# liangxuy/ReGenNet

Measured on AMD Instinct MI355X. Metric: sampled motions/sec, higher is better.
Workload: dtype bf16 MFMA operands, fp32 accumulate/LayerNorm/softmax, for 990 of 1000 steps; fp16 MFMA operands for the next 8; split-bf16 (x3) for the last 2; 1 GPU; ntu: [B=256/GPU,56,6,60] online/concat/no_cond L8 d512, 1000-step DDPM, Philox noise, hipGraph=on; batch_per_gpu=256, global_batch=256, denoiser_evals_per_motion=1000, parallelism=batch-shard x1

## Files before the change

regennet_amd/csrc/rgn_layers.hip:

```cpp
#include "rgn_internal.h"
#include "rgn_device.h"
#include "rgn_tail.h"
#include "rgn_sampler.h"

#include <hip/hip_runtime.h>

#include <cmath>
#include <type_traits>
#include <utility>

namespace rgn {

#ifndef RGN_LY_ST_AUX
#define RGN_LY_ST_AUX 16
#endif

constexpr int LY_NTH = 512, LY_KB = 4096;
constexpr int LY_X = 0, LY_Y = 64 * 1024, LY_EXCH = LY_Y, LY_RED = 128 * 1024, LY_REDF = 2 * 8 * 64, LY_VEC = LY_RED + 2 * LY_REDF * 4, LY_VECW = 640,
              LY_LDS = 160 * 1024;
constexpr int LY_PF = LY_VEC + 8 * LY_VECW * 4;
static_assert(LY_PF + 8 * 256 <= LY_LDS, "LDS map");
enum { V_BO = 0, V_G1 = 64, V_G2 = 128, V_B2 = 192, V_SPV = 256, V_BF1 = 320 , V_BF2 = 448, V_G3 = 512, V_B3 = 576 };
constexpr int LY_RDA = 6;
constexpr int LY_RDM = 8;
struct LYT {
    static constexpr int MT = 2, NT = 2, NW = 8, R = 64, RD = LY_RDM, KB = LY_KB, RED = LY_RED, REDF = LY_REDF;
};

#ifdef RGN_LY_STAMPS
__device__ long long g_ly_st[1024][16];
#define RGN_LYT(i)                                                                                   \
    {                                                                                                \
        __builtin_amdgcn_sched_barrier(0);                                                           \
        if (threadIdx.x == 0 && blockIdx.x < 1024 && l == RGN_LY_STAMPS) g_ly_st[blockIdx.x][i] = __builtin_readcyclecounter(); \
        __builtin_amdgcn_sched_barrier(0);                                                           \
    }
#define RGN_LYS(i)                                                                                   \
    {                                                                                                \
        __builtin_amdgcn_sched_barrier(0);                                                           \
        if (threadIdx.x == 0 && blockIdx.x < 1024 && it == 1) g_ly_st[blockIdx.x][i] = __builtin_readcyclecounter(); \
        __builtin_amdgcn_sched_barrier(0);                                                           \
    }
#else
#define RGN_LYT(i)
#define RGN_LYS(i)
#endif

constexpr int LY_XLD = 356, LY_TILE = 0, LY_XIMG = 92160, LY_NKX = 11;
static_assert(64 * LY_XLD * 4 <= LY_XIMG && LY_XIMG + LY_NKX * 4096 <= LY_LDS, "step boundary LDS map");

template <bool STEPS, bool GUIDED = false, bool F16 = false, bool INPAINT = false>
__global__ __launch_bounds__(LY_NTH, 2) void k_layers(LayersArgs g) {
    static_assert(STEPS || !GUIDED, "guidance inside the launch needs the step boundary");
    static_assert(STEPS || !INPAINT, "in-painting (rgn_set_inpainting) belongs to the step boundary");
    using OP = OpFmt<F16>;
    using op_t = typename OP::t;
    using op8 = typename OP::v8;
    using op4 = typename OP::v4;
    extern __shared__ __attribute__((aligned(16))) char smem[];
    const int tid = threadIdx.x, lane = tid & 63;
    const int wave = __builtin_amdgcn_readfirstlane(tid >> 6);
    const int wn = wave & 3, hg = wave >> 2;
    const int l31 = lane & 31, kh = lane >> 5;
    const int b = xcd_affine(blockIdx.x, gridDim.x), Tq = g.Tq;
    const size_t row0 = (size_t)b * Tq;
#ifdef RGN_LY_PRIO
    if (wave >= 4) __builtin_amdgcn_s_setprio(RGN_LY_PRIO);
#endif
    float* vec = reinterpret_cast<float*>(smem + LY_VEC) + wave * LY_VECW;
    const int lane16 = lane * 16;
    tile_dma_in(smem + LY_X, g.h, g.rows, row0, Tq, lane, wave);
    const int first_step = (g.stepvec || STEPS) ? *g.d_step : 0;
    const TailLane tl = tail_lane<LYT>(smem, lane, wave);
    static_assert(LY_X == 0, "a_off addresses the image at byte 0");
    int a_off[2], a_offy[2];
    tail_a_off(a_off, lane);
    tail_a_off(a_offy, a_off, LY_Y);
    using Pass = TailPass;
    op8 wf[LY_RDM][2];
    const float qs2 = g.qscale * 1.44269504088896340736f;

    f32x4 qb[4];
    float vb1;
    auto load_qbias = [&](const float* bqkv, int r) {
        const float* bq = bqkv + (2 * r + hg) * 128 + wn * 32;
#pragma unroll
        for (int i4 = 0; i4 < 4; ++i4) qb[i4] = *reinterpret_cast<const f32x4*>(bq + 8 * i4 + 4 * kh);
        vb1 = bq[1024 + l31];
    };

    wait_vmcnt<0>();
    __builtin_amdgcn_s_barrier();
    load_qbias(g.lw[0].bqkv, 0);

    const int nit = STEPS ? g.steps : 1;
    auto out_proj = [&](f32x16 (&acc)[2][2], int wv) {
#pragma unroll
        for (int a2 = 0; a2 < 2; ++a2)
#pragma unroll
            for (int b2 = 0; b2 < 2; ++b2)
#pragma unroll
                for (int i = 0; i < 16; ++i) acc[a2][b2][i] = 0.f;
        if (wv < 6) {
            const int cb0 = 2 * wv;
            const Pass p_out{__builtin_amdgcn_make_buffer_rsrc(const_cast<__bf16*>(g.Wout) + (size_t)cb0 * 1024, 0, (16 * g.nb_out - cb0) * 2048, 0x00020000), LY_NKX * 2048, 0};
#pragma unroll
            for (int s2 = 0; s2 < LY_RDM - 1; ++s2) tail_load_g<OP, LYT>(wf, tl, p_out, s2, s2);
            tail_gemm<OP, LYT, 32, false, 0>(acc, wf, tl, a_off, p_out, p_out);
        }
    };
    for (int it = 0; it < nit; ++it) {
    const int step = first_step - it;
    for (int pass = 0; pass < (GUIDED ? 2 : 1); ++pass) {
    if (GUIDED && pass == 1) {
        f32x16 accp[2][2];
        int wave_p = wave, lane_p = lane, b_p = b;
        asm volatile("" : "+s"(wave_p), "+s"(b_p));
        asm volatile("" : "+v"(lane_p));
        out_proj(accp, wave_p);
        if (wave_p < 6) {
            float* pk = g.park + ((size_t)b_p * 6 + wave_p) * 4096 + lane_p * 4;
#pragma unroll
            for (int nt = 0; nt < 2; ++nt)
#pragma unroll
                for (int mt = 0; mt < 2; ++mt)
#pragma unroll
                    for (int i4 = 0; i4 < 4; ++i4)
                        *reinterpret_cast<f32x4*>(pk + ((nt * 2 + mt) * 4 + i4) * 256) = f32x4{accp[nt][mt][4 * i4], accp[nt][mt][4 * i4 + 1], accp[nt][mt][4 * i4 + 2], accp[nt][mt][4 * i4 + 3]};
        }
        __builtin_amdgcn_s_barrier();
        tile_dma_in<16>(smem + LY_X, g.h, g.rows, g.half + (size_t)b_p * Tq, Tq, lane_p, wave_p);
        wait_vmcnt<0>();
        __builtin_amdgcn_s_barrier();
    }
    for (int l = 0; l < g.L; ++l) {
        const LayerWts& w = g.lw[l];
        RGN_LYT(0)
        op4 attk[2][2][4];
        float bo_r = 0.f;
        {
            struct PassA { __amdgpu_buffer_rsrc_t rs; };
            auto qrs = [&](int r) {
                const int blk = (2 * r + hg) * 4 + wn;
                return __builtin_amdgcn_make_buffer_rsrc(const_cast<__bf16*>(w.Wqkv) + (size_t)blk * 1024, 0, 3 * 512 * 512 * 2 - blk * 2048, 0x00020000);
            };
            const PassA pa[2] = {{qrs(0)}, {qrs(1)}};
            op8 wq[LY_RDA][3];
            auto load_ga = [&](const PassA& ps, int hs, int slot) {
                int soff;
                asm volatile("s_mov_b32 %0, %1" : "=s"(soff) : "i"(frag_granule(hs, 48 * 2048)));
#pragma unroll
                for (int t = 0; t < 3; ++t)
                    wq[slot][t] = __builtin_bit_cast(op8, __builtin_amdgcn_raw_buffer_load_b128(ps.rs, lane16, soff + t * (16 * 2048), 0));
            };
            constexpr int AH = LY_RDA - 1;
#pragma unroll
            for (int s = 0; s < AH; ++s) load_ga(pa[0], s, s);
#pragma unroll
            for (int r = 0; r < 2; ++r) {
                const int head = 2 * r + hg;
                f32x16 acc[2][3];
#pragma unroll
                for (int ta = 0; ta < 2; ++ta)
#pragma unroll
                    for (int i4 = 0; i4 < 4; ++i4)
#pragma unroll
                        for (int e = 0; e < 4; ++e) {
                            acc[ta][0][4 * i4 + e] = qb[i4][e];
                            acc[ta][1][4 * i4 + e] = 0.f;
                            acc[ta][2][4 * i4 + e] = vb1;
                        }
                __builtin_amdgcn_sched_barrier(0);
                {
                    op8 af[2];
#pragma unroll
                    for (int ta = 0; ta < 2; ++ta) af[ta] = *reinterpret_cast<const op8*>(smem + a_off[0] + ta * 2048);
#pragma unroll
                    for (int hs = 0; hs < 32; ++hs) {
                        op8 afn[2];
#pragma unroll
                        for (int ta = 0; ta < 2; ++ta) {
                            afn[ta] = af[ta];
                            if (hs + 1 < 32) afn[ta] = *reinterpret_cast<const op8*>(smem + ((hs + 1) >> 1) * LY_KB + a_off[(hs + 1) & 1] + ta * 2048);
                        }
                        if (hs + AH < 32) load_ga(pa[r], hs + AH, (32 * r + hs + AH) % LY_RDA);
                        else if (r == 0) load_ga(pa[1], hs + AH - 32, (32 * r + hs + AH) % LY_RDA);
                        if (hs + AH < 32 || r == 0) {
                            if (hs < AH) wait_vmcnt<3 * AH + 5>();
                            else wait_vmcnt<3 * AH>();
                        }
                        const int slot = (32 * r + hs) % LY_RDA;
#pragma unroll
                        for (int t = 0; t < 3; ++t)
#pragma unroll
                            for (int ta = 0; ta < 2; ++ta) {
                                if (t < 2) acc[ta][t] = OP::mfma(wq[slot][t], af[ta], acc[ta][t]);
                                else acc[ta][t] = OP::mfma(af[ta], wq[slot][t], acc[ta][t]);
                            }
#pragma unroll
                        for (int ta = 0; ta < 2; ++ta) af[ta] = afn[ta];
                    }
                }
                __builtin_amdgcn_sched_barrier(0);
                RGN_LYT(1 + 3 * r)
                op8 qh[2][2], kf[2][2], vh[2][2];
#pragma unroll
                for (int ta = 0; ta < 2; ++ta)
#pragma unroll
                    for (int sl = 0; sl < 2; ++sl)
#pragma unroll
                        for (int j = 0; j < 8; ++j) {
                            const int i = 8 * sl + j;
                            qh[ta][sl][j] = (op_t)acc[ta][0][i];
                            kf[ta][sl][j] = (op_t)acc[ta][1][i];
                            vh[ta][sl][j] = (op_t)acc[ta][2][i];
                        }
                if (r == 0) load_qbias(w.bqkv, 1);
                else bo_r = w.bo[64 * wave + lane];
                f32x16 st[3];
#pragma unroll
                for (int tl = 0; tl < 3; ++tl) {
                    const int kj = tl >> 1, qtile = tl ? 1 : 0;
#pragma unroll
                    for (int i = 0; i < 16; ++i) st[tl][i] = 0.f;
#pragma unroll
                    for (int sl = 0; sl < 2; ++sl) st[tl] = OP::mfma(kf[kj][sl], qh[qtile][sl], st[tl]);
                }
                f32x4* sred = reinterpret_cast<f32x4*>(smem + LY_EXCH);
#pragma unroll
                for (int tl = 0; tl < 3; ++tl)
#pragma unroll
                    for (int i4 = 0; i4 < 4; ++i4) {
                        const f32x4 v = {st[tl][4 * i4], st[tl][4 * i4 + 1], st[tl][4 * i4 + 2], st[tl][4 * i4 + 3]};
                        sred[(((hg * 3 + tl) * 4 + wn) * 4 + i4) * 64 + lane] = v;
                    }
                if (r == 0) { RGN_LYT(12) }
                wait_lgkmcnt<0>();
                __builtin_amdgcn_s_barrier();
                if (r == 0) { RGN_LYT(13) }
                {
                    const int kg = lane & 3, qi = lane >> 2, qt = qi >> 3, ql = 8 * wn + (qi & 7), Q = 32 * qt + ql;
                    const int kj = kg >> 1, sl = kg & 1;
                    const bool live = !(qt == 0 && kj == 1);
                    const int tl = live ? qt + kj : 0;
                    const char* ex = smem + LY_EXCH + ((hg * 3 + tl) * 4 * 4 + 2 * sl) * 1024 + ql * 16;
                    f32x4 sv[4];
#pragma unroll
                    for (int a2 = 0; a2 < 2; ++a2)
#pragma unroll
                        for (int h2 = 0; h2 < 2; ++h2) {
                            f32x4 v = *reinterpret_cast<const f32x4*>(ex + a2 * 1024 + h2 * 512);
#pragma unroll
                            for (int ww = 1; ww < 4; ++ww) {
                                const f32x4 u = *reinterpret_cast<const f32x4*>(ex + ww * 4096 + a2 * 1024 + h2 * 512);
#pragma unroll
                                for (int e = 0; e < 4; ++e) v[e] += u[e];
                            }
                            sv[2 * a2 + h2] = v;
                        }
                    int xlim = live ? (Q < Tq - 1 ? Q : Tq - 1) - 32 * kj - 16 * sl : -1;
                    asm volatile("" : "+v"(xlim));
                    float mx = -INFINITY;
#pragma unroll
                    for (int c4 = 0; c4 < 4; ++c4)
#pragma unroll
                        for (int e = 0; e < 4; ++e) {
                            sv[c4][e] = (4 * c4 + e <= xlim) ? sv[c4][e] : -INFINITY;
                            mx = fmaxf(mx, sv[c4][e]);
                        }
                    mx = fmaxf(mx, __builtin_bit_cast(float, __builtin_amdgcn_mov_dpp(__builtin_bit_cast(int, mx), 0xB1, 0xf, 0xf, true)));
                    mx = fmaxf(mx, __builtin_bit_cast(float, __builtin_amdgcn_mov_dpp(__builtin_bit_cast(int, mx), 0x4E, 0xf, 0xf, true)));
                    float sum = 0.f;
                    const float nmx = -mx * qs2;
#pragma unroll
                    for (int c4 = 0; c4 < 4; ++c4)
#pragma unroll
                        for (int e = 0; e < 4; ++e) {
                            sv[c4][e] = __builtin_amdgcn_exp2f(__builtin_fmaf(sv[c4][e], qs2, nmx));
                            sum += sv[c4][e];
                        }
                    sum += __builtin_bit_cast(float, __builtin_amdgcn_mov_dpp(__builtin_bit_cast(int, sum), 0xB1, 0xf, 0xf, true));
                    sum += __builtin_bit_cast(float, __builtin_amdgcn_mov_dpp(__builtin_bit_cast(int, sum), 0x4E, 0xf, 0xf, true));
                    const float inv = 1.0f / sum;
                    if (live) {
#pragma unroll
                        for (int h2 = 0; h2 < 2; ++h2) {
                            op8 pp;
#pragma unroll
                            for (int e = 0; e < 4; ++e) {
                                pp[e] = (op_t)(sv[h2][e] * inv);
                                pp[4 + e] = (op_t)(sv[2 + h2][e] * inv);
                            }
                            *reinterpret_cast<op8*>(smem + LY_EXCH + (((hg * 3 + tl) * 4 + 0) * 4 + sl) * 1024 + (h2 * 32 + ql) * 16) = pp;
                        }
                    }
                }
                if (r == 0) { RGN_LYT(14) }
                wait_lgkmcnt<0>();
                __builtin_amdgcn_s_barrier();
                if (r == 0) { RGN_LYT(15) }
#pragma unroll
                for (int qtile = 0; qtile < 2; ++qtile) {
                    f32x16 oa;
#pragma unroll
                    for (int i = 0; i < 16; ++i) oa[i] = 0.f;
#pragma unroll
                    for (int tl = qtile; tl <= 2 * qtile; ++tl) {
                        const int kj = tl >> 1;
#pragma unroll
                        for (int sl = 0; sl < 2; ++sl) {
                            const op8 ph = *reinterpret_cast<const op8*>(smem + LY_EXCH + (((hg * 3 + tl) * 4 + 0) * 4 + sl) * 1024 + lane * 16);
                            oa = OP::mfma(vh[kj][sl], ph, oa);
                        }
                    }
#pragma unroll
                    for (int i4 = 0; i4 < 4; ++i4)
#pragma unroll
                        for (int e = 0; e < 4; ++e) attk[r][qtile][i4][e] = (op_t)oa[4 * i4 + e];
                }
                RGN_LYT(2 + 3 * r)
                wait_lgkmcnt<0>();
                __builtin_amdgcn_s_barrier();
                RGN_LYT(3 + 3 * r)
            }
        }
        const Pass p_wo{tail_wrs(w.Wo, 2 * wave, 512 * 512 * 2), 16 * 2048, 0}, p_w1a{tail_wrs(w.W1, 2 * wave, 1024 * 512 * 2), 32 * 2048, 0},
            p_w1b{tail_wrs(w.W1, 16 + 2 * wave, 1024 * 512 * 2), 32 * 2048, 0}, p_w2a{tail_wrs(w.W2, 2 * wave, 512 * 1024 * 2), 16 * 2048, 0},
            p_w2b{p_w2a.rs, 16 * 2048, 32};
        vec[V_BO + lane] = bo_r;
#pragma unroll
        for (int s = 0; s < LY_RDM - 1; ++s) tail_load_g<OP, LYT>(wf, tl, p_wo, s, s);
        int cw = 64 * wave + lane;
        asm volatile("" : "+v"(cw));
        float vv[12];
        {
            const float* src[9] = {w.bo, w.g1, w.g2, w.b2, w.bf1, w.bf1 + 512, w.bf2, w.g3, w.b3};
            vv[1] = src[1][cw]; vv[2] = src[2][cw]; vv[3] = src[3][cw];
            vv[4] = w.b1[cw] + (g.stepvec ? g.stepvec[(size_t)step * g.ldstep + (size_t)l * 512 + cw] : 0.f) +
                    (g.pervec ? g.pervec[((size_t)b + (size_t)pass * g.B) * g.ldper + (size_t)l * 512 + cw] : 0.f);
            vv[5] = src[4][cw]; vv[6] = src[5][cw]; vv[7] = src[6][cw]; vv[8] = src[7][cw]; vv[9] = src[8][cw];
        }
        asm volatile("" ::: "memory");
#pragma unroll
        for (int r = 0; r < 2; ++r)
#pragma unroll
            for (int qtile = 0; qtile < 2; ++qtile)
#pragma unroll
                for (int i4 = 0; i4 < 4; ++i4)
                    *reinterpret_cast<op4*>(smem + LY_Y + ((2 * r + hg) * 4 + wn) * LY_KB + (32 * qtile + l31) * 64 + img_slot(i4, tl.swz) + 8 * kh) = attk[r][qtile][i4];
        wait_lgkmcnt<0>();
        __builtin_amdgcn_s_barrier();
        f32x16 acc[2][2];
        tail_init_bias<LYT>(acc, tl, vec + V_BO);
        RGN_LYT(7)
        tail_gemm<OP, LYT, 32, true, 11>(acc, wf, tl, a_offy, p_wo, p_w1a);
        RGN_LYT(8)
        vec[V_G1 + lane] = vv[1]; vec[V_G2 + lane] = vv[2]; vec[V_B2 + lane] = vv[3]; vec[V_SPV + lane] = vv[4];
        vec[V_BF1 + lane] = vv[5]; vec[V_BF1 + 64 + lane] = vv[6]; vec[V_BF2 + lane] = vv[7]; vec[V_G3 + lane] = vv[8]; vec[V_B3 + lane] = vv[9];
        tail_add_resid<OP, LYT>(acc, tl, LY_X);
        tail_layernorm<LYT, 0>(acc, tl, vec + V_G1, tail_rowvec(tl, vec + V_SPV));
        tail_layernorm<LYT, 1>(acc, tl, vec + V_G2, tail_rowvec(tl, vec + V_B2));
        tail_store_img<OP, LYT>(acc, tl, LY_X);
        wait_lgkmcnt<0>();
        __builtin_amdgcn_s_barrier();
        RGN_LYT(9)
        f32x16 acc2[2][2];
        tail_ffn<OP, LYT>(acc2, wf, tl, a_off, a_offy, LY_Y, p_w1a, p_w1b, p_w2a, p_w2b, vec + V_BF1, vec + V_BF2);
        load_qbias(g.lw[l + 1 < g.L ? l + 1 : 0].bqkv, 0);
#ifndef RGN_LY_NO_PREFETCH
        if constexpr (STEPS) {
            if (l == g.L - 1) {
                const int nsl = (int)(gridDim.x >> 3) >= 32 ? 32 : ((int)(gridDim.x >> 3) > 0 ? (int)(gridDim.x >> 3) : 1);
                const int sl = (int)(blockIdx.x >> 3) % nsl;
                const int n_out = 16 * g.nb_out * 16, n_all = n_out + LY_NKX * 16 * 16;
                const unsigned pf_lds = (unsigned)(size_t)((RGN_AS3 char*)(smem + LY_PF)) + (unsigned)wave * 256u;
                for (int ln = sl + nsl * tid; ln < n_all; ln += nsl * LY_NTH) {
                    const char* pp = ln < n_out ? reinterpret_cast<const char*>(g.Wout) + (size_t)ln * 128 : reinterpret_cast<const char*>(g.Wx) + (size_t)(ln - n_out) * 128;
                    int m0_keep;
                    asm volatile("s_mov_b32 %0, m0\n\ts_mov_b32 m0, %2\n\ts_nop 0\n\tglobal_load_lds_dword %1, off\n\ts_mov_b32 m0, %0" : "=&s"(m0_keep) : "v"(pp), "s"(pf_lds) : "memory");
                }
            }
        }
#endif
        RGN_LYT(10)
        tail_add_resid<OP, LYT>(acc2, tl, LY_X);
        tail_layernorm<LYT, 0>(acc2, tl, vec + V_G3, tail_rowvec(tl, vec + V_B3));
        tail_store_img<OP, LYT>(acc2, tl, LY_X);
        wait_lgkmcnt<0>();
        __builtin_amdgcn_s_barrier();
        RGN_LYT(11)
    }
    }
    if constexpr (STEPS) {
        int lane_s = lane, wave_s = wave, b_s = b;
        asm volatile("" : "+v"(lane_s));
        asm volatile("" : "+s"(wave_s), "+s"(b_s));
        const int l31_s = lane_s & 31, kh_s = lane_s >> 5;
        const size_t row0_s = (size_t)b_s * Tq;
        auto col4s = [&](int nt, int i4) { return 32 * nt + 8 * i4 + 4 * kh_s; };
        RGN_LYS(12)
        const SampleParams sp = *g.sp;
        const StepCoef k = g.tab[step];
        const int T = Tq, gb = g.s0 + b_s;
        const float gscale = GUIDED ? g.scale[gb] : 0.f;
        const __amdgpu_buffer_rsrc_t park_rs = __builtin_amdgcn_make_buffer_rsrc(GUIDED ? g.park + ((size_t)b_s * 6 + (wave_s < 6 ? wave_s : 0)) * 4096 : nullptr, 0, 4096 * 4, 0x00020000);
        f32x16 acc[2][2];
        out_proj(acc, wave_s);
        __builtin_amdgcn_s_barrier();
        float* tile = reinterpret_cast<float*>(smem + LY_TILE);
#pragma unroll
        for (int nt = 0; nt < 2; ++nt)
#pragma unroll
            for (int i4 = 0; i4 < 4; ++i4) {
                const int n = 64 * wave_s + col4s(nt, i4);
                if (n < 352) {
                    f32x4 bb = {0.f, 0.f, 0.f, 0.f};
                    if (n < g.F) bb = *reinterpret_cast<const f32x4*>(g.bout + n);
#pragma unroll
                    for (int mt = 0; mt < 2; ++mt) {
                        f32x4 v = {acc[nt][mt][4 * i4] + bb[0], acc[nt][mt][4 * i4 + 1] + bb[1], acc[nt][mt][4 * i4 + 2] + bb[2], acc[nt][mt][4 * i4 + 3] + bb[3]};
                        if constexpr (GUIDED) {
                            const f32x4 cc = __builtin_bit_cast(f32x4, __builtin_amdgcn_raw_buffer_load_b128(park_rs, (lane_s * 4 + ((nt * 2 + mt) * 4 + i4) * 256) * 4, 0, 16));
#pragma unroll
                            for (int e = 0; e < 4; ++e) v[e] = guide(cc[e] + bb[e], v[e], gscale);
                        }
                        *reinterpret_cast<f32x4*>(tile + (32 * mt + l31_s) * LY_XLD + n) = v;
                    }
                }
            }
        const Pass p_wx{__builtin_amdgcn_make_buffer_rsrc(const_cast<__bf16*>(g.Wx) + (size_t)(2 * wave_s) * 1024, 0, (LY_NKX * 16 - 2 * wave_s) * 2048, 0x00020000), 16 * 2048, 0};
#pragma unroll
        for (int s2 = 0; s2 < LY_RDM - 1; ++s2) tail_load_g<OP, LYT>(wf, tl, p_wx, s2, s2);
        op4 c0v[2][2][4];
#pragma unroll
        for (int mt = 0; mt < 2; ++mt) {
            const int r = 32 * mt + l31_s, rr = r < T ? r : T - 1;
#pragma unroll
            for (int nt = 0; nt < 2; ++nt)
#pragma unroll
                for (int i4 = 0; i4 < 4; ++i4)
                    c0v[nt][mt][i4] = *reinterpret_cast<const op4*>(g.c0 + (row0_s + rr) * 512 + 64 * wave_s + col4s(nt, i4));
        }
        op4 c0u[GUIDED ? 2 : 1][2][4];
        if constexpr (GUIDED) {
#pragma unroll
            for (int mt = 0; mt < 2; ++mt) {
                const int r = 32 * mt + l31_s, rr = r < T ? r : T - 1;
#pragma unroll
                for (int nt = 0; nt < 2; ++nt)
#pragma unroll
                    for (int i4 = 0; i4 < 4; ++i4)
                        c0u[nt][mt][i4] = *reinterpret_cast<const op4*>(g.c0 + ((size_t)g.half + row0_s + rr) * 512 + 64 * wave_s + col4s(nt, i4));
            }
        }
        wait_lgkmcnt<0>();
        __builtin_amdgcn_s_barrier();
        RGN_LYS(13)
        {
            const int t = lane_s;
            const bool valid = t < T;
            const size_t FT = (size_t)g.F * T;
            const int bn = noise_motion(sp, gb);
            char* ximg = smem + LY_XIMG;
            const int q = lane_s & 3, tq = t - q;
            const bool run4 = valid && (tq & 3) == 0 && tq + 3 < T;
            const bool quads = !sp.noise && !g.no_quads && __all(run4 || tq >= T);
            float xpre[LY_NKX][4];
#pragma unroll
            for (int i2 = 0; i2 < LY_NKX; ++i2)
#pragma unroll
                for (int j = 0; j < 4; ++j) {
                    const int f = 4 * (wave_s + 8 * i2) + j;
                    xpre[i2][j] = (valid && f < g.F) ? sp.x[(size_t)gb * FT + (size_t)f * T + t] : 0.f;
                }
            const int ximg_lane = img_run(lane_s, wave_s >> 1, wave_s & 1);
            constexpr int LY_IPD = GUIDED ? 1 : 2;
            unsigned char mpre[INPAINT ? LY_NKX : 1][4];
            float ipre[INPAINT ? LY_NKX : 1][4];
            const InpaintRsrc irs = inpaint_rsrc(sp, INPAINT ? (size_t)gb * FT : 0, INPAINT ? FT : 0);
            auto inp_request = [&](auto IG) __attribute__((always_inline)) {
                constexpr int ig = decltype(IG)::value;
                if constexpr (INPAINT && ig < LY_NKX) {
#pragma unroll
                    for (int j = 0; j < 4; ++j) inpaint_load(irs, t, (4 * (wave_s + 8 * ig) + j) * T, mpre[ig][j], ipre[ig][j]);
                    asm volatile("" ::: "memory");
                }
            };
            static_for<LY_IPD>([&](auto IG) __attribute__((always_inline)) { inp_request(IG); });
            auto update4 = [&](int i2, int fg, const float (&eps_in)[4], const float (&xv)[4]) {
                op4 nvb;
#pragma unroll
                for (int j = 0; j < 4; ++j) nvb[j] = (op_t)0.f;
                if (valid && 4 * fg < g.F) {
                    const f32x4 x04 = *reinterpret_cast<const f32x4*>(tile + lane_s * LY_XLD + 4 * fg);
#pragma unroll
                    for (int j = 0; j < 4; ++j) {
                        const int f = 4 * fg + j;
                        unsigned char im = 0;
                        float iv = 0.f;
                        if constexpr (INPAINT) { im = mpre[i2][j]; iv = ipre[i2][j]; }
                        const float x0 = pred_x0<INPAINT>(x04[j], im, iv, sp.clip);
                        const size_t o = (size_t)gb * FT + (size_t)f * T + t;
                        if (sp.x0_out) sp.x0_out[o] = x0;
                        const float nv = sampler_next(k, sp.sampler, x0, xv[j], quad_or_step_eps(quads, eps_in[j], sp, step, g.B, FT, bn, f, T, t));
                        sp.x[o] = nv;
                        nvb[j] = (op_t)nv;
                    }
                }
                *reinterpret_cast<op4*>(ximg + i2 * 4096 + ximg_lane) = nvb;
            };
            static_for<LY_NKX>([&](auto IT) __attribute__((always_inline)) {
                constexpr int i2 = decltype(IT)::value;
                const int fg = wave_s + 8 * i2;
                inp_request(std::integral_constant<int, i2 + LY_IPD>{});
                float eps4[4] = {0.f, 0.f, 0.f, 0.f};
                if (quads) quad_normals(sp, step, bn, fg, q, tq, eps4);
                update4(i2, fg, eps4, xpre[i2]);
            });
        }
        wait_lgkmcnt<0>();
        __builtin_amdgcn_s_barrier();
        RGN_LYS(14)
#pragma unroll
        for (int a2 = 0; a2 < 2; ++a2)
#pragma unroll
            for (int b2 = 0; b2 < 2; ++b2)
#pragma unroll
                for (int i = 0; i < 16; ++i) acc[a2][b2][i] = 0.f;
        {
            int a_offx[2] = {a_off[0] + LY_XIMG, a_off[1] + LY_XIMG};
            tail_gemm<OP, LYT, 2 * LY_NKX, false, 8 + 16>(acc, wf, tl, a_offx, p_wx, p_wx);
        }
        if constexpr (GUIDED) {
            __builtin_amdgcn_s_barrier();
#pragma unroll
            for (int nt = 0; nt < 2; ++nt)
#pragma unroll
                for (int i4 = 0; i4 < 4; ++i4)
#pragma unroll
                    for (int mt = 0; mt < 2; ++mt) {
                        op4 hh;
#pragma unroll
                        for (int e = 0; e < 4; ++e) hh[e] = (op_t)(acc[nt][mt][4 * i4 + e] + (float)c0u[nt][mt][i4][e]);
                        *tail_img_run<OP, LYT>(tl, LY_Y, nt, i4, mt) = hh;
                    }
        }
#pragma unroll
        for (int nt = 0; nt < 2; ++nt)
#pragma unroll
            for (int mt = 0; mt < 2; ++mt)
#pragma unroll
                for (int i4 = 0; i4 < 4; ++i4)
#pragma unroll
                    for (int e = 0; e < 4; ++e) acc[nt][mt][4 * i4 + e] += (float)c0v[nt][mt][i4][e];
        tail_store_img<OP, LYT>(acc, tl, LY_X);
        wait_lgkmcnt<0>();
        __builtin_amdgcn_s_barrier();
        if constexpr (GUIDED) {
            const __amdgpu_buffer_rsrc_t u_rs = __builtin_amdgcn_make_buffer_rsrc(g.out, 0, (int)((size_t)g.rows * 512 * 2), 0x00020000);
            const int r16 = lane_s >> 2, c = lane_s & 3;
#pragma unroll
            for (int j = 0; j < 8; ++j) {
                const int p = wave_s * 8 + j, blk = p >> 2, r = (p & 3) * 16 + r16;
                if (r < T) {
                    const int off = blk * LY_KB + r * 64 + ((c ^ ((r >> 2) & 3)) << 4);
                    __builtin_amdgcn_raw_buffer_store_b128(*reinterpret_cast<const u32x4*>(smem + LY_Y + off), u_rs,
                                                           (int)((((size_t)blk * g.rows + g.half + row0_s + r) * 32 + c * 8) * 2), 0, RGN_LY_ST_AUX);
                }
            }
        }
        RGN_LYS(15)
    }
    }
    {
        const __amdgpu_buffer_rsrc_t o_rs = __builtin_amdgcn_make_buffer_rsrc(g.out, 0, (int)((size_t)g.rows * 512 * 2), 0x00020000);
        const int r16 = lane >> 2, c = lane & 3;
#pragma unroll
        for (int j = 0; j < 8; ++j) {
            const int p = wave * 8 + j, blk = p >> 2, r = (p & 3) * 16 + r16;
            if (r < Tq) {
                const int off = blk * LY_KB + img_chunk(r, c);
                __builtin_amdgcn_raw_buffer_store_b128(*reinterpret_cast<const u32x4*>(smem + LY_X + off), o_rs,
                                                       (int)(plane_chunk(g.rows, row0 + r, blk, c) * 2), 0, RGN_LY_ST_AUX);
            }
        }
    }
    if constexpr (STEPS) {
        if (tid == 0) step_ticket(g.d_stepw + 4, (int)gridDim.x, g.d_stepw, first_step - g.steps);
    }
}

#ifdef RGN_LY_STAMPS
void ly_stamps_read(long long* out) { (void)hipMemcpyFromSymbol(out, HIP_SYMBOL(g_ly_st), sizeof(long long) * 1024 * 16); }
#endif

bool layers_supported(int d, int ff, int H, int Tq, int L) { return d == 512 && ff == 1024 && H == 4 && Tq >= 1 && Tq <= 64 && L >= 1 && L <= LY_MAXL; }
bool layers_steps_supported(int d, int F, int Kpx) { return d == 512 && F % 4 == 0 && F <= 352 && Kpx == 32 * LY_NKX; }
constexpr bool layers_form_exists(bool steps, bool guided, bool inpaint) { return steps || !(guided || inpaint); }
template <class Fn>
static hipError_t layers_form(bool steps, bool guided, bool f16, bool inpaint, Fn fn) {
    return dispatch_bools([&](auto S, auto G, auto H, auto I) {
        if constexpr (layers_form_exists(decltype(S)::value, decltype(G)::value, decltype(I)::value))
            return fn(k_layers<decltype(S)::value, decltype(G)::value, decltype(H)::value, decltype(I)::value>);
        else
            return hipErrorInvalidValue;
    }, steps, guided, f16, inpaint);
}
hipError_t configure_layers() {
    hipError_t e = hipSuccess;
    for (int m = 0; m < 16 && e == hipSuccess; ++m)
        if (layers_form_exists(m & 1, m & 2, m & 8))
            e = layers_form(m & 1, m & 2, m & 4, m & 8, [](auto kern) { return hipFuncSetAttribute(reinterpret_cast<const void*>(kern), hipFuncAttributeMaxDynamicSharedMemorySize, LY_LDS); });
    return e;
}
hipError_t launch_layers(const LayersArgs& g, hipStream_t s, bool inpaint) {
    const bool steps = g.steps > 0;
    return layers_form(steps, steps && g.scale, g.f16 != 0, inpaint, [&](auto kern) {
        hipLaunchKernelGGL(kern, dim3(g.Bm), dim3(LY_NTH), LY_LDS, s, g);
        return hipGetLastError();
    });
}

}
```

Baseline: 462.9 motions/s.

## Split sampler update into pipelined quad path and rolled fallback with buffer ops

The fused sampler-update tail now separates the fast quad-noise path from the fallback. The quad path uses raw buffer loads and stores with an out-of-range offset to mask invalid lanes. It software-pipelines the x and inpaint loads two groups ahead in a rolled loop. The generic path becomes a compact rolled per-element loop that calls step_eps directly. The aim is to cut register pressure and code size from the fully unrolled prefetch of every group while keeping memory latency hidden, at the cost of less unrolling and reliance on buffer out-of-bounds behaviour for masking.

```diff
diff --git a/regennet_amd/csrc/rgn_layers.hip b/regennet_amd/csrc/rgn_layers.hip
--- a/regennet_amd/csrc/rgn_layers.hip
+++ b/regennet_amd/csrc/rgn_layers.hip
@@ -465,58 +465,86 @@
             const int q = lane_s & 3, tq = t - q;
             const bool run4 = valid && (tq & 3) == 0 && tq + 3 < T;
             const bool quads = !sp.noise && !g.no_quads && __all(run4 || tq >= T);
-            float xpre[LY_NKX][4];
-#pragma unroll
-            for (int i2 = 0; i2 < LY_NKX; ++i2)
-#pragma unroll
-                for (int j = 0; j < 4; ++j) {
-                    const int f = 4 * (wave_s + 8 * i2) + j;
-                    xpre[i2][j] = (valid && f < g.F) ? sp.x[(size_t)gb * FT + (size_t)f * T + t] : 0.f;
-                }
             const int ximg_lane = img_run(lane_s, wave_s >> 1, wave_s & 1);
-            constexpr int LY_IPD = GUIDED ? 1 : 2;
-            unsigned char mpre[INPAINT ? LY_NKX : 1][4];
-            float ipre[INPAINT ? LY_NKX : 1][4];
             const InpaintRsrc irs = inpaint_rsrc(sp, INPAINT ? (size_t)gb * FT : 0, INPAINT ? FT : 0);
-            auto inp_request = [&](auto IG) __attribute__((always_inline)) {
-                constexpr int ig = decltype(IG)::value;
-                if constexpr (INPAINT && ig < LY_NKX) {
-#pragma unroll
-                    for (int j = 0; j < 4; ++j) inpaint_load(irs, t, (4 * (wave_s + 8 * ig) + j) * T, mpre[ig][j], ipre[ig][j]);
+            if (quads) {
+                constexpr int LY_NOSTORE = 0x7ffffff0;
+                static_assert(LY_NKX % 2 == 1, "pairs of groups, then the last one");
+                const __amdgpu_buffer_rsrc_t x_rs = __builtin_amdgcn_make_buffer_rsrc(sp.x + (size_t)gb * FT, 0, (int)(FT * 4), 0x00020000);
+                const __amdgpu_buffer_rsrc_t x0_rs = __builtin_amdgcn_make_buffer_rsrc(sp.x0_out ? sp.x0_out + (size_t)gb * FT : nullptr, 0, sp.x0_out ? (int)(FT * 4) : 0, 0x00020000);
+                struct Grp {
+                    float x[4];
+                    unsigned char m[INPAINT ? 4 : 1];
+                    float iv[INPAINT ? 4 : 1];
+                };
+                auto request = [&](int i2, Grp& r) __attribute__((always_inline)) {
+                    const int e0 = 4 * (wave_s + 8 * i2) * T + t;
+#pragma unroll
+                    for (int j = 0; j < 4; ++j) {
+                        r.x[j] = __builtin_bit_cast(float, __builtin_amdgcn_raw_buffer_load_b32(x_rs, (e0 + j * T) * 4, 0, 0));
+                        if constexpr (INPAINT) inpaint_load(irs, e0 + j * T, 0, r.m[j], r.iv[j]);
+                    }
+                };
+                auto group = [&](int i2, const Grp& r) __attribute__((always_inline)) {
+                    const int fg = wave_s + 8 * i2;
+                    float eps4[4];
+                    quad_normals(sp, step, bn, fg, q, tq, eps4);
+                    const bool ok = valid && 4 * fg < g.F;
+                    const int e0 = 4 * fg * T + t;
+                    const f32x4 x04 = *reinterpret_cast<const f32x4*>(tile + lane_s * LY_XLD + 4 * fg);
+                    op4 nvb;
+#pragma unroll
+                    for (int j = 0; j < 4; ++j) {
+                        unsigned char im = 0;
+                        float iv = 0.f;
+                        if constexpr (INPAINT) { im = r.m[j]; iv = r.iv[j]; }
+                        const float x0 = pred_x0<INPAINT>(x04[j], im, iv, sp.clip);
+                        const int off = ok ? (e0 + j * T) * 4 : LY_NOSTORE;
+                        if (sp.x0_out) __builtin_amdgcn_raw_buffer_store_b32(__builtin_bit_cast(int, x0), x0_rs, off, 0, 0);
+                        const float nv = sampler_next(k, sp.sampler, x0, r.x[j], eps4[j]);
+                        __builtin_amdgcn_raw_buffer_store_b32(__builtin_bit_cast(int, nv), x_rs, off, 0, 0);
+                        nvb[j] = ok ? (op_t)nv : (op_t)0.f;
+                    }
+                    *reinterpret_cast<op4*>(ximg + i2 * 4096 + ximg_lane) = nvb;
+                };
+                Grp ra, rb, rc, rd;
+                request(0, ra);
+                request(1, rb);
+#pragma unroll 1
+                for (int i2 = 0; i2 < LY_NKX - 1; i2 += 2) {
+                    request(i2 + 2, rc);
+                    request(i2 + 3, rd);
                     asm volatile("" ::: "memory");
-                }
-            };
-            static_for<LY_IPD>([&](auto IG) __attribute__((always_inline)) { inp_request(IG); });
-            auto update4 = [&](int i2, int fg, const float (&eps_in)[4], const float (&xv)[4]) {
-                op4 nvb;
-#pragma unroll
-                for (int j = 0; j < 4; ++j) nvb[j] = (op_t)0.f;
-                if (valid && 4 * fg < g.F) {
-                    const f32x4 x04 = *reinterpret_cast<const f32x4*>(tile + lane_s * LY_XLD + 4 * fg);
-#pragma unroll
+                    group(i2, ra);
+                    group(i2 + 1, rb);
+                    ra = rc;
+                    rb = rd;
+                }
+                group(LY_NKX - 1, ra);
+            } else {
+#pragma unroll 1
+                for (int i2 = 0; i2 < LY_NKX; ++i2) {
+                    const int fg = wave_s + 8 * i2;
+                    const bool ok = valid && 4 * fg < g.F;
+#pragma unroll 1
                     for (int j = 0; j < 4; ++j) {
                         const int f = 4 * fg + j;
-                        unsigned char im = 0;
-                        float iv = 0.f;
-                        if constexpr (INPAINT) { im = mpre[i2][j]; iv = ipre[i2][j]; }
-                        const float x0 = pred_x0<INPAINT>(x04[j], im, iv, sp.clip);
-                        const size_t o = (size_t)gb * FT + (size_t)f * T + t;
-                        if (sp.x0_out) sp.x0_out[o] = x0;
-                        const float nv = sampler_next(k, sp.sampler, x0, xv[j], quad_or_step_eps(quads, eps_in[j], sp, step, g.B, FT, bn, f, T, t));
-                        sp.x[o] = nv;
-                        nvb[j] = (op_t)nv;
-                    }
-                }
-                *reinterpret_cast<op4*>(ximg + i2 * 4096 + ximg_lane) = nvb;
-            };
-            static_for<LY_NKX>([&](auto IT) __attribute__((always_inline)) {
-                constexpr int i2 = decltype(IT)::value;
-                const int fg = wave_s + 8 * i2;
-                inp_request(std::integral_constant<int, i2 + LY_IPD>{});
-                float eps4[4] = {0.f, 0.f, 0.f, 0.f};
-                if (quads) quad_normals(sp, step, bn, fg, q, tq, eps4);
-                update4(i2, fg, eps4, xpre[i2]);
-            });
+                        float nv = 0.f;
+                        if (ok) {
+                            unsigned char im = 0;
+                            float iv = 0.f;
+                            if constexpr (INPAINT) inpaint_load(irs, f * T + t, 0, im, iv);
+                            const float x0 = pred_x0<INPAINT>(tile[lane_s * LY_XLD + f], im, iv, sp.clip);
+                            const size_t o = (size_t)gb * FT + (size_t)f * T + t;
+                            if (sp.x0_out) sp.x0_out[o] = x0;
+                            nv = sampler_next(k, sp.sampler, x0, sp.x[o], step_eps(sp, step, g.B, FT, bn, f, T, t));
+                            sp.x[o] = nv;
+                        }
+                        *reinterpret_cast<op_t*>(ximg + i2 * 4096 + ximg_lane + j * (int)sizeof(op_t)) = (op_t)nv;
+                    }
+                }
+                __builtin_amdgcn_s_waitcnt(0x0070);
+            }
         }
         wait_lgkmcnt<0>();
         __builtin_amdgcn_s_barrier();
```

Result: no change. 467.4 motions/s (median of 6 runs) (+1.0%).
